# s3prl/s3prl

Hardware: AMD Instinct MI355X
Metric: encoder-frames/sec (20 ms stride) HuBERT-base 32x10 s @16 kHz (higher is better)
Workload: dtype f32; 1 GPU; hubert_base random-init, 32x10 s @16 kHz per GPU, one UpstreamExpert.forward per step: all 13 hidden_states (fp32) written; utterances_per_gpu=32, global_batch=32, samples=160000, frames_per_utt=499, parallelism=dp1, lengths=equal, gather=none

## Files before the change

### include/s3enc.h

```cpp
#ifndef S3ENC_H
#define S3ENC_H

#include <stdint.h>

#ifdef __cplusplus
extern "C" {
#endif

#define S3ENC_VERSION 8
#define S3ENC_MAX_CONV 16
#define S3ENC_MAX_RES 4

typedef struct s3enc_encoder* s3enc_handle;

enum { S3ENC_HUBERT = 0, S3ENC_WAV2VEC2 = 1, S3ENC_WAVLM = 2,
       S3ENC_DISTILLER = 3,
       S3ENC_MULTIRES = 4,
       S3ENC_WAV2VEC = 5,
       S3ENC_CPC = 6,
       S3ENC_APC = 7,
       S3ENC_MOCKINGJAY = 8,
       S3ENC_DECOAR = 9,
       S3ENC_NPC = 10 };
enum { S3ENC_F32 = 0, S3ENC_BF16 = 1, S3ENC_F16 = 2,
// ... 171 lines not shown
    const float* feat_w;
} s3enc_forward_opts;
int s3enc_num_states(s3enc_handle h, int32_t selection, int32_t* n);
int s3enc_forward_ex(s3enc_handle h, const float* const* wavs, const int64_t* lengths, int32_t B, int64_t n_max,
                     const s3enc_forward_opts* opts, void* out, int64_t layer_stride, void* stream);

int s3enc_forward_aux(s3enc_handle h, const float* const* wavs, const int64_t* lengths, int32_t B, int64_t n_max,
                      const s3enc_forward_opts* opts, void* out, int64_t layer_stride, float* codewords, int64_t* codeids,
                      void* stream);

enum { S3ENC_STATUS_NONFINITE = 1, S3ENC_STATUS_PENDING = 1 << 30 };
int s3enc_forward_status(s3enc_handle h, int32_t wait, int32_t* status);

int s3enc_set_layer_events(s3enc_handle h, void* const* events, int32_t n);

typedef struct s3enc_comm_s* s3enc_comm;
int s3enc_comm_version(int32_t* version);
int s3enc_comm_unique_id(void* id128);
int s3enc_comm_init_rank(const void* id128, int32_t world, int32_t rank, int32_t device, s3enc_comm* out);
int s3enc_comm_info(s3enc_comm c, int32_t* world, int32_t* rank);
int s3enc_comm_allgather_states(s3enc_comm c, const void* send, int64_t send_state_stride, void* recv, int64_t recv_state_stride,
                                int32_t n_states, int64_t bytes_per_state, void* const* ready_events, void* stream);
#define S3ENC_EXCHANGE_COLLECTIVE 0
#define S3ENC_EXCHANGE_DIRECT 1
#define S3ENC_EXCHANGE_COPY 2
#define S3ENC_COPY_HANDLE_BYTES 256
int s3enc_comm_init_local(int32_t world, int32_t rank, int32_t device, s3enc_comm* out);
int s3enc_comm_copy_export(s3enc_comm c, void* recv_slab, int64_t bytes, void* handle_out);
int s3enc_comm_copy_attach(s3enc_comm c, const void* handles );
int s3enc_comm_copy_status(s3enc_comm c, int32_t* status);
int s3enc_comm_copy_release(s3enc_comm c, void* stream);
int s3enc_comm_exchange_states(s3enc_comm c, int32_t algo, const void* send, int64_t send_state_stride, void* recv,
                               int64_t recv_state_stride, int32_t n_states, int64_t bytes_per_state, void* const* ready_events,
                               void* stream);
int s3enc_comm_destroy(s3enc_comm c);

int s3enc_forward_padded(s3enc_handle h, const float* pcm, int64_t row_stride, const int64_t* lengths, int32_t B,
                         int64_t n_max, float* out, int64_t layer_stride, void* stream);

int s3enc_profile_enable(s3enc_handle h, int32_t on);
int s3enc_profile_reset(s3enc_handle h);
typedef struct s3enc_profile_entry {
    char name[48];
    int64_t launches;
    double ms;
    double flops;
    double bytes;
} s3enc_profile_entry;
int s3enc_profile_read(s3enc_handle h, s3enc_profile_entry* entries, int32_t max_entries, int32_t* n_entries);

int s3enc_debug_tap(s3enc_handle h, const char* name, float* host_out, int64_t max_elems, int64_t* n_elems);
int s3enc_debug_occupy_cus(int32_t workgroups, int32_t threads, double milliseconds, void* stream);
int s3enc_debug_clock_sample(uint64_t* out3_device, void* stream);

int s3enc_set_tuning(const char* key, int32_t value);
int s3enc_set_handle_tuning(s3enc_handle h, const char* key, int32_t value);


int s3enc_op_gemm(int32_t dtype, const void* A, int64_t lda, int64_t a_batch_stride, const void* W,
                  const float* bias, int32_t M, int32_t N, int32_t K, int32_t batches, int32_t act,
                  const float* residual, const int32_t* row_limit, float* out32, void* out16, int64_t ldo,
                  int64_t o_batch_stride, void* stream);

int s3enc_op_conv0(int32_t dtype, const float* const* wavs, const int64_t* lengths, int32_t B, int64_t n_max,
                   int32_t normalize, const float* w0, const float* bias, const float* gn_gamma, const float* gn_beta,
                   const float* ln_gamma, const float* ln_beta, int32_t C, int32_t stride, void* out, void* stream);
int s3enc_op_wavlm_gate(const float* x, const float* grep_w, const float* grep_b, const float* grep_a, int32_t B, int32_t T,
                        int32_t H, float* gate, void* stream);

int s3enc_op_layernorm(int32_t dtype, const float* x, const float* gamma, const float* beta, int32_t rows,
                       int32_t C, int32_t act, float* out32, void* out16, void* stream);

int s3enc_op_attention(int32_t dtype, const void* qkv, void* out, const int32_t* valid, int32_t B, int32_t T,
                       int32_t H, const float* bias_table, int32_t table_R, const float* gate, void* stream);

int s3enc_op_conformer_conv(const float* x, const float* taps, const float* shift, int32_t B, int32_t T, int32_t D, int32_t K,
                            float* out, void* stream);
int s3enc_op_relpos_attention(const float* qkv, float* out, const int32_t* valid, int32_t B, int32_t T, int32_t H, const float* P,
                              const float* qadd, void* stream);

int s3enc_op_gn1_apply(const float* x, const float* gamma, const float* beta, const float* res, float scale, int32_t log_compress,
                       int32_t B, int32_t rows, int32_t C, int32_t pad, int32_t pad_zero, float* dst, float* state, float* acc,
                       float acc_w, int32_t acc_norm, int32_t acc_init, void* stream);
int s3enc_op_argmax_gather(const float* scores, const float* table, int32_t shared, int64_t rows, int32_t G, int32_t V, int32_t Dv,
                           int64_t* ids, float* out, void* stream);

int s3enc_op_channelnorm_relu(const float* x, const float* gamma, const float* beta, int32_t B, int32_t rows, int32_t C,
                              int32_t pad, float* dst, float* state, void* stream);
int s3enc_op_rnn(int32_t cell, const float* pre, const float* w_hh_host, const float* b_hn, int32_t B, int32_t T, int32_t H,
                 int64_t ld_pre, float* out, int64_t ldo, void* stream);

int s3enc_op_rnn_len(int32_t cell, const float* pre, const float* w_hh_host, const float* b_hn, const int32_t* len_host,
                     const float* res, int64_t ld_res, int32_t B, int32_t T, int32_t H, int64_t ld_pre, float* out, int64_t ldo,
                     void* stream);

int s3enc_op_conv_taps(const float* x, const float* w_host, const float* bias, int32_t B, int32_t T, int32_t C, int32_t N, int32_t k,
                       int32_t mask, int32_t act, const float* res, int64_t ld_res, float* dst, int32_t dst_pad, int64_t ldo,
                       float* state, float* sum, int32_t sum_init, int32_t dense, void* stream);

int s3enc_op_lstm_bidir(const float* pre_fwd, const float* pre_bwd, const float* w_hh_fwd_host, const float* w_hh_bwd_host,
                        const int32_t* len_host, int32_t B, int32_t T, int32_t H, int64_t ld_pre, float* out, int64_t ldo,
                        void* stream);
int s3enc_pack_lstm_bidir_whh(const float* w_hh_host, int32_t H, float* out_host);

int s3enc_op_posconv(int32_t dtype, const float* x, const float* w_host, const float* bias, int32_t B, int32_t T, int32_t D,
                     int32_t G, int32_t K, float* out, void* stream);
// ... 38 lines not shown
```

### s3prl_amd/_lib.py

```python

from __future__ import annotations

import ctypes as C
import os

_HERE = os.path.dirname(os.path.abspath(__file__))
LIB_PATH = os.path.join(_HERE, "libs3enc.so")

S3ENC_MAX_CONV = 16
S3ENC_MAX_RES = 4
F32, BF16, F16, F32X3, F16X2 = 0, 1, 2, 3, 4
STATUS_NONFINITE, STATUS_PENDING = 1, 1 << 30
DTYPES = {"fp32": F32, "f32": F32, "float32": F32, "bf16": BF16, "bfloat16": BF16, "fp16": F16, "f16": F16,
          "float16": F16, "fp32x3": F32X3, "f32x3": F32X3, "bf16x3": F32X3,
          "fp16x2": F16X2, "f16x2": F16X2}
FAMILY = {"hubert": 0, "wav2vec2": 1, "wavlm": 2, "distiller": 3, "multires_hubert": 4, "wav2vec": 5, "cpc": 6, "apc": 7, "mockingjay": 8, "decoar": 9, "npc": 10}
CPC_NORM = {"layerNorm": 0, "instanceNorm": 1, "ID": 2, "batchNorm": 3}
CPC_AR = {"LSTM": 0, "GRU": 1, "RNN": 2, "transformer": 3, "no_ar": 4}
APC_WINDOW = {"povey": 0, "hamming": 1}
VQ_TYPE = {"none": 0, "gumbel": 1, "kmeans": 2}
SEL_HIDDEN, SEL_LAYER_OUT, SEL_FFN_OUT = 0, 1, 2
SELECTIONS = {None: SEL_HIDDEN, "hidden_states": SEL_HIDDEN, "fairseq_layers": SEL_LAYER_OUT,
              "fairseq_layers_before_residual": SEL_FFN_OUT}
ABI_VERSION = 8
# ... 85 lines not shown

class S3FbankConfig(C.Structure):
    _fields_ = [("sample_rate", C.c_int32), ("num_mel_bins", C.c_int32), ("frame_length_ms", C.c_float),
                ("frame_shift_ms", C.c_float), ("preemphasis", C.c_float), ("delta_order", C.c_int32),
                ("delta_win_length", C.c_int32), ("use_cmvn", C.c_int32), ("cmvn_eps", C.c_float)]


_VP, _I32, _I64 = C.c_void_p, C.c_int32, C.c_int64
_PROTOS = {
    "s3enc_version": (C.c_int, []),
    "s3enc_last_error": (C.c_char_p, []),
    "s3enc_create": (C.c_int, [C.POINTER(S3Config), C.POINTER(S3Tensor), _I32, _I32, C.POINTER(_VP)]),
    "s3enc_create_ex": (C.c_int, [C.POINTER(S3Config), C.POINTER(S3Wav2vecConfig), C.POINTER(S3Tensor), _I32, _I32, C.POINTER(_VP)]),
    "s3enc_create_cpc": (C.c_int, [C.POINTER(S3Config), C.POINTER(S3CpcConfig), C.POINTER(S3Tensor), _I32, _I32, C.POINTER(_VP)]),
    "s3enc_create_apc": (C.c_int, [C.POINTER(S3Config), C.POINTER(S3ApcConfig), C.POINTER(S3Tensor), _I32, _I32, C.POINTER(_VP)]),
    "s3enc_create_mockingjay": (C.c_int, [C.POINTER(S3Config), C.POINTER(S3MockingjayConfig), C.POINTER(S3Tensor), _I32, _I32,
                                          C.POINTER(_VP)]),
    "s3enc_create_decoar": (C.c_int, [C.POINTER(S3Config), C.POINTER(S3DecoarConfig), C.POINTER(S3Tensor), _I32, _I32, C.POINTER(_VP)]),
    "s3enc_create_npc": (C.c_int, [C.POINTER(S3Config), C.POINTER(S3NpcConfig), C.POINTER(S3Tensor), _I32, _I32, C.POINTER(_VP)]),
    "s3enc_destroy": (C.c_int, [_VP]),
    "s3enc_num_frames": (C.c_int, [_VP, _I64, C.POINTER(_I32)]),
    "s3enc_num_output_frames": (C.c_int, [_VP, _I64, C.POINTER(_I32)]),
    "s3enc_downsample_rate": (C.c_int, [_VP, C.POINTER(_I32)]),
    "s3enc_valid_frames": (C.c_int, [_VP, _I64, _I64, C.POINTER(_I32)]),
    "s3enc_forward": (C.c_int, [_VP, C.POINTER(_VP), C.POINTER(_I64), _I32, _I64, _VP, _I64, _VP]),
    "s3enc_forward_status": (C.c_int, [_VP, _I32, C.POINTER(_I32)]),
    "s3enc_forward_ex": (C.c_int, [_VP, C.POINTER(_VP), C.POINTER(_I64), _I32, _I64, C.POINTER(S3ForwardOpts), _VP, _I64, _VP]),
    "s3enc_forward_aux": (C.c_int, [_VP, C.POINTER(_VP), C.POINTER(_I64), _I32, _I64, C.POINTER(S3ForwardOpts), _VP, _I64, _VP, _VP, _VP]),
    "s3enc_num_states": (C.c_int, [_VP, _I32, C.POINTER(_I32)]),
    "s3enc_forward_padded": (C.c_int, [_VP, _VP, _I64, C.POINTER(_I64), _I32, _I64, _VP, _I64, _VP]),
    "s3enc_set_layer_events": (C.c_int, [_VP, C.POINTER(_VP), _I32]),
    "s3enc_profile_enable": (C.c_int, [_VP, _I32]),
    "s3enc_profile_reset": (C.c_int, [_VP]),
    "s3enc_profile_read": (C.c_int, [_VP, C.POINTER(S3ProfileEntry), _I32, C.POINTER(_I32)]),
    "s3enc_debug_tap": (C.c_int, [_VP, C.c_char_p, C.POINTER(C.c_float), _I64, C.POINTER(_I64)]),
    "s3enc_comm_version": (C.c_int, [C.POINTER(_I32)]),
    "s3enc_comm_unique_id": (C.c_int, [_VP]),
    "s3enc_comm_init_rank": (C.c_int, [_VP, _I32, _I32, _I32, C.POINTER(_VP)]),
    "s3enc_comm_info": (C.c_int, [_VP, C.POINTER(_I32), C.POINTER(_I32)]),
    "s3enc_comm_allgather_states": (C.c_int, [_VP, _VP, _I64, _VP, _I64, _I32, _I64, C.POINTER(_VP), _VP]),
    "s3enc_comm_exchange_states": (C.c_int, [_VP, _I32, _VP, _I64, _VP, _I64, _I32, _I64, C.POINTER(_VP), _VP]),
    "s3enc_comm_destroy": (C.c_int, [_VP]),
    "s3enc_comm_init_local": (C.c_int, [_I32, _I32, _I32, C.POINTER(_VP)]),
    "s3enc_comm_copy_export": (C.c_int, [_VP, _VP, _I64, _VP]),
    "s3enc_comm_copy_attach": (C.c_int, [_VP, _VP]),
    "s3enc_comm_copy_status": (C.c_int, [_VP, C.POINTER(_I32)]),
    "s3enc_comm_copy_release": (C.c_int, [_VP, _VP]),
    "s3enc_set_handle_tuning": (C.c_int, [_VP, C.c_char_p, _I32]),
    "s3enc_set_tuning": (C.c_int, [C.c_char_p, _I32]),
    "s3enc_op_gemm": (C.c_int, [_I32, _VP, _I64, _I64, _VP, _VP, _I32, _I32, _I32, _I32, _I32, _VP, _VP, _VP, _VP,
                                _I64, _I64, _VP]),
    "s3enc_debug_occupy_cus": (C.c_int, [_I32, _I32, C.c_double, _VP]),
    "s3enc_debug_clock_sample": (C.c_int, [_VP, _VP]),
    "s3enc_op_layernorm": (C.c_int, [_I32, _VP, _VP, _VP, _I32, _I32, _I32, _VP, _VP, _VP]),
    "s3enc_op_attention": (C.c_int, [_I32, _VP, _VP, _VP, _I32, _I32, _I32, _VP, _I32, _VP, _VP]),
    "s3enc_op_conv0": (C.c_int, [_I32, C.POINTER(_VP), C.POINTER(_I64), _I32, _I64, _I32, _VP, _VP, _VP, _VP, _VP, _VP, _I32,
                                 _I32, _VP, _VP]),
    "s3enc_op_wavlm_gate": (C.c_int, [_VP, _VP, _VP, _VP, _I32, _I32, _I32, _VP, _VP]),
    "s3enc_op_conformer_conv": (C.c_int, [_VP, _VP, _VP, _I32, _I32, _I32, _I32, _VP, _VP]),
    "s3enc_op_gn1_apply": (C.c_int, [_VP, _VP, _VP, _VP, C.c_float, _I32, _I32, _I32, _I32, _I32, _I32, _VP, _VP, _VP, C.c_float,
                                     _I32, _I32, _VP]),
    "s3enc_op_channelnorm_relu": (C.c_int, [_VP, _VP, _VP, _I32, _I32, _I32, _I32, _VP, _VP, _VP]),
    "s3enc_op_rnn": (C.c_int, [_I32, _VP, _VP, _VP, _I32, _I32, _I32, _I64, _VP, _I64, _VP]),
    "s3enc_op_rnn_len": (C.c_int, [_I32, _VP, _VP, _VP, _VP, _VP, _I64, _I32, _I32, _I32, _I64, _VP, _I64, _VP]),
    "s3enc_op_lstm_bidir": (C.c_int, [_VP, _VP, _VP, _VP, _VP, _I32, _I32, _I32, _I64, _VP, _I64, _VP]),
    "s3enc_pack_lstm_bidir_whh": (C.c_int, [_VP, _I32, _VP]),
    "s3enc_op_conv_taps": (C.c_int, [_VP, _VP, _VP, _I32, _I32, _I32, _I32, _I32, _I32, _I32, _VP, _I64, _VP, _I32, _I64, _VP, _VP,
                                     _I32, _I32, _VP]),
    "s3enc_op_argmax_gather": (C.c_int, [_VP, _VP, _I32, _I64, _I32, _I32, _I32, _VP, _VP, _VP]),
    "s3enc_op_relpos_attention": (C.c_int, [_VP, _VP, _VP, _I32, _I32, _I32, _VP, _VP, _VP]),
    "s3enc_op_posconv": (C.c_int, [_I32, _VP, _VP, _VP, _I32, _I32, _I32, _I32, _I32, _VP, _VP]),
    "s3enc_weighted_sum": (C.c_int, [_VP, _I64, _I32, C.POINTER(C.c_float), _I32, _I64, _I32, _VP, _VP]),
    "s3enc_weighted_sum_backward_scratch": (_I64, [_I64, _I32]),
    "s3enc_weighted_sum_backward": (C.c_int, [_VP, _I64, _I32, _I32, _I64, _I32, _VP, _VP, _VP, _VP]),
    "s3enc_fbank_num_frames": (C.c_int, [C.POINTER(S3FbankConfig), _I64, C.POINTER(_I32)]),
    "s3enc_fbank_forward": (C.c_int, [C.POINTER(S3FbankConfig), _VP, C.POINTER(_I64), _I32, _VP, _I64, _I32, _VP]),
    "s3enc_fbank_forward_ex": (C.c_int, [C.POINTER(S3FbankConfig), _I32, _VP, C.POINTER(_I64), _I32, _VP, _I64, _I32, _VP]),
    "s3enc_logmel_frame_counts": (C.c_int, [C.POINTER(_I64), _I32, _I64, C.POINTER(_I32)]),
    "s3enc_logmel_forward": (C.c_int, [_VP, C.POINTER(_I64), _I32, _I64, _I32, C.c_float, _I32, C.POINTER(_I32), _VP, _I32, _VP]),
    "s3enc_op_layernorm_eps": (C.c_int, [_VP, _VP, _VP, C.c_float, _I64, _I32, _VP, _VP]),
    "s3enc_op_input_repr": (C.c_int, [_VP, _VP, _VP, _VP, _I32, _VP, _VP, C.c_float, _I64, _I32, _I32, _VP, _VP]),
}

_lib = None


class S3EncError(RuntimeError):
    pass


def load():
    global _lib
    if _lib is not None:
        return _lib
    if not os.path.exists(LIB_PATH):
        raise S3EncError(
            f"{LIB_PATH} not found — build it with `python -c 'import __graft_entry__ as g; g.build()'` "
            f"or `make -C s3prl_amd/csrc`.  There is no CPU / PyTorch fallback for the encoder path."
        )
    try:
        import torch
    except Exception:
        pass
    lib = C.CDLL(LIB_PATH, mode=C.RTLD_GLOBAL)
    for name, (res, args) in _PROTOS.items():
        fn = getattr(lib, name)
# ... 164 lines not shown
```

### s3prl_amd/csrc/gemmt.hip

```cpp
#include <type_traits>

#include "kernels.h"

namespace s3 {

namespace {

constexpr int BN = 128, ROWB = 64;
typedef int i32x4 __attribute__((ext_vector_type(4)));

struct x3_tag {};
template <typename T> struct TileElem { typedef typename Cvt<T>::store_t type; };
template <> struct TileElem<x3_tag> { typedef float type; };

template <typename T> struct TileMma;
template <> struct TileMma<float> {
    static __device__ __forceinline__ void run(const uint4& a, const uint4& b, f32x16& c) {
        c = __builtin_amdgcn_mfma_f32_32x32x2f32(__uint_as_float(a.x), __uint_as_float(b.x), c, 0, 0, 0);
        c = __builtin_amdgcn_mfma_f32_32x32x2f32(__uint_as_float(a.y), __uint_as_float(b.y), c, 0, 0, 0);
        c = __builtin_amdgcn_mfma_f32_32x32x2f32(__uint_as_float(a.z), __uint_as_float(b.z), c, 0, 0, 0);
        c = __builtin_amdgcn_mfma_f32_32x32x2f32(__uint_as_float(a.w), __uint_as_float(b.w), c, 0, 0, 0);
    }
};
template <> struct TileMma<bf16_tag> {
    static __device__ __forceinline__ void run(const uint4& a, const uint4& b, f32x16& c) {
        c = __builtin_amdgcn_mfma_f32_32x32x16_bf16(__builtin_bit_cast(bf16x8, a), __builtin_bit_cast(bf16x8, b), c, 0, 0, 0);
    }
};
template <typename T, int TM>
__global__ __launch_bounds__(256, 2) void gemm_tile_kernel(GemmParams p) {
    typedef typename TileElem<T>::type store_t;
    constexpr int EB = sizeof(store_t);
    constexpr bool X3 = std::is_same<T, x3_tag>::value;
    constexpr int BM = 64 * TM;
    constexpr int PLANE = (BM + BN) * ROWB;
    constexpr int NPASS = (BM + BN) / 64;
    constexpr int APASS = BM / 64;
    extern __shared__ __attribute__((aligned(16))) char smem[];
    const int tid = threadIdx.x;
    const int lane = tid & 63;
    const int wave = __builtin_amdgcn_readfirstlane(tid >> 6);
    const int wr = wave >> 1, wc = wave & 1;
    const int half = lane >> 5;
    const int l31 = lane & 31;

    const int n_tiles = (p.N + BN - 1) / BN;
    const int m_tiles = (p.M + BM - 1) / BM;
    int tile;
    {
        const int nwg = gridDim.x, wg = blockIdx.x;
        const int q8 = nwg >> 3, r8 = nwg & 7, xcd = wg & 7, loc = wg >> 3;
        tile = (xcd < r8 ? xcd * (q8 + 1) : r8 * (q8 + 1) + (xcd - r8) * q8) + loc;
    }
    const int tn = tile % n_tiles;
    const int tmb = tile / n_tiles;
    const int tm = tmb % m_tiles, b = tmb / m_tiles;
    const int m0 = tm * BM, n0 = tn * BN;
    const int nk = (p.K * EB) >> 6;

    i32x4 rsrc_a, rsrc_w;
    {
        const char* ab = (const char*)p.A + (long)b * p.a_bs * EB;
        const unsigned long ua = (unsigned long)ab, uw = (unsigned long)(X3 ? p.W_x3 : p.W);
        rsrc_a = (i32x4){(int)__builtin_amdgcn_readfirstlane((unsigned)ua), (int)__builtin_amdgcn_readfirstlane((unsigned)(ua >> 32)),
                         -1, 0x00020000};
        rsrc_w = (i32x4){(int)__builtin_amdgcn_readfirstlane((unsigned)uw), (int)__builtin_amdgcn_readfirstlane((unsigned)(uw >> 32)),
                         -1, 0x00020000};
    }
    const int src_slot = (lane & 3) ^ ((lane >> 4) & 3);
    unsigned voff[NPASS];
#pragma unroll
    for (int i = 0; i < NPASS; ++i) {
        if (i < APASS) {
            int r = m0 + 16 * wave + 64 * i + (lane >> 2);
            r = r < p.M ? r : p.M - 1;
            voff[i] = (unsigned)r * (unsigned)(p.lda * EB) + src_slot * 16;
        } else {
            int r = n0 + 16 * wave + 64 * (i - APASS) + (lane >> 2);
            r = r < p.N ? r : p.N - 1;
            voff[i] = (unsigned)r * (unsigned)(p.K * EB) + src_slot * 16;
        }
    }
    const unsigned lds0 = __builtin_amdgcn_readfirstlane((unsigned)(uintptr_t)(__attribute__((address_space(3))) char*)smem) + wave * 1024;
    auto dma = [&](unsigned vo, const i32x4& rs, unsigned dst, unsigned soff) {
        asm volatile("s_mov_b32 m0, %0\n\ts_nop 0\n\tbuffer_load_dwordx4 %1, %2, %3 offen lds"
                     :
                     : "s"(dst), "v"(vo), "s"(rs), "s"(soff)
                     : "memory");
    };
    auto issue = [&](int kt, int slot) {
        const unsigned kb = (unsigned)kt * ROWB;
        const unsigned d0 = lds0 + slot * PLANE;
#pragma unroll
        for (int i = 0; i < NPASS; ++i) dma(voff[i], i < APASS ? rsrc_a : rsrc_w, d0 + i * 4096, kb);
    };

    const int swz = (l31 >> 2) & 3;
    const char* fa_base = smem + (wr * (TM * 32) + l31) * ROWB;
    const char* fb_base = smem + (BM + wc * 64 + l31) * ROWB;
    const int so0 = ((half * 2) ^ swz) << 4, so1 = ((half * 2 + 1) ^ swz) << 4;

    f32x16 acc[TM][2];
#pragma unroll
    for (int i = 0; i < TM; ++i)
#pragma unroll
        for (int j = 0; j < 2; ++j)
#pragma unroll
            for (int r = 0; r < 16; ++r) acc[i][j][r] = 0.f;

    struct Frag {
        uint4 a[TM], b[2];
    };
    auto read = [&](Frag& f, int slot, int so) {
#pragma unroll
        for (int i = 0; i < TM; ++i) f.a[i] = *(const uint4*)(fa_base + slot * PLANE + i * 32 * ROWB + so);
#pragma unroll
        for (int j = 0; j < 2; ++j) f.b[j] = *(const uint4*)(fb_base + slot * PLANE + j * 32 * ROWB + so);
    };
    issue(0, 0);
    asm volatile("s_waitcnt vmcnt(0)" ::: "memory");
    __builtin_amdgcn_s_barrier();
    asm volatile("" ::: "memory");
    if (nk > 1) issue(1, 1);
    if constexpr (!X3) {
        auto mma = [&](const Frag& f, int i, int j) { TileMma<T>::run(f.a[i], f.b[j], acc[i][j]); };
        auto mma_all = [&](const Frag& f) {
#pragma unroll
            for (int i = 0; i < TM; ++i)
#pragma unroll
                for (int j = 0; j < 2; ++j) mma(f, i, j);
        };
        Frag f0, f1;
        read(f0, 0, so0);
        auto step = [&](int kt, int slot) {
            read(f1, slot, so1);
            mma_all(f0);
            __builtin_amdgcn_sched_barrier(0);
            asm volatile("s_waitcnt vmcnt(0) lgkmcnt(0)" ::: "memory");
            __builtin_amdgcn_s_barrier();
            asm volatile("" ::: "memory");
            __builtin_amdgcn_sched_barrier(0);
            mma(f1, 0, 0);
            __builtin_amdgcn_sched_barrier(0);
            if (kt + 2 < nk) issue(kt + 2, slot);
            if (kt + 1 < nk) read(f0, slot ^ 1, so0);
            __builtin_amdgcn_sched_barrier(0);
#pragma unroll
            for (int i = 0; i < TM; ++i)
#pragma unroll
                for (int j = 0; j < 2; ++j)
                    if (i | j) mma(f1, i, j);
        };
        int kt = 0;
        for (; kt + 1 < nk; kt += 2) {
            step(kt, 0);
            step(kt + 1, 1);
        }
        if (kt < nk) step(kt, 0);
    } else {
        auto mma_row = [&](const Frag& lo_half, const Frag& hi_half, int i) {
            uint4 ah, al;
            split8(__builtin_bit_cast(float4, lo_half.a[i]), __builtin_bit_cast(float4, hi_half.a[i]), ah, al);
#pragma unroll
            for (int j = 0; j < 2; ++j) {
                TileMma<bf16_tag>::run(al, lo_half.b[j], acc[i][j]);
                TileMma<bf16_tag>::run(ah, hi_half.b[j], acc[i][j]);
                TileMma<bf16_tag>::run(ah, lo_half.b[j], acc[i][j]);
            }
        };
        Frag f0, f1, g0, g1;
        read(f0, 0, so0);
        read(f1, 0, so1);
        auto step = [&](int kt, int slot, Frag& c0, Frag& c1, Frag& n0_, Frag& n1_) {
            mma_row(c0, c1, 0);
            __builtin_amdgcn_sched_barrier(0);
            asm volatile("s_waitcnt vmcnt(0) lgkmcnt(0)" ::: "memory");
            __builtin_amdgcn_s_barrier();
            asm volatile("" ::: "memory");
            __builtin_amdgcn_sched_barrier(0);
            if (kt + 2 < nk) issue(kt + 2, slot);
            if (kt + 1 < nk) {
                read(n0_, slot ^ 1, so0);
                read(n1_, slot ^ 1, so1);
            }
            __builtin_amdgcn_sched_barrier(0);
#pragma unroll
            for (int i = 1; i < TM; ++i) mma_row(c0, c1, i);
        };
        int kt = 0;
        for (; kt + 1 < nk; kt += 2) {
            step(kt, 0, f0, f1, g0, g1);
            step(kt + 1, 1, g0, g1, f0, f1);
        }
        if (kt < nk) step(kt, 0, f0, f1, g0, g1);
    }

    const int limit = p.row_limit ? p.row_limit[b] : p.M;
    const long ob = (long)b * p.o_bs;
    float* stg = (float*)(smem + wave * 8192);
    {
        const int c4 = (lane & 15) * 4;
        const int n = n0 + wc * 64 + c4;
        const bool n_ok = n < p.N;
        float4 bias4 = make_float4(0.f, 0.f, 0.f, 0.f);
        if (p.bias && n_ok) bias4 = *(const float4*)(p.bias + n);
#pragma unroll
        for (int i = 0; i < TM; ++i) {
#pragma unroll
            for (int j = 0; j < 2; ++j)
#pragma unroll
                for (int r = 0; r < 16; ++r) stg[((r & 3) + 8 * (r >> 2) + 4 * half) * 64 + j * 32 + l31] = acc[i][j][r];
            asm volatile("s_waitcnt lgkmcnt(0)" ::: "memory");
#pragma unroll
            for (int t = 0; t < 8; ++t) {
                const int row = t * 4 + (lane >> 4);
                float4 v = *(const float4*)(stg + row * 64 + c4);
                const int m = m0 + wr * (TM * 32) + i * 32 + row;
                if (m < p.M && n_ok) {
                    v.x += bias4.x; v.y += bias4.y; v.z += bias4.z; v.w += bias4.w;
                    if (p.act == 3) {
                        swish4(v);
                    } else if (p.act) {
                        if (X3 || p.act == 2) {
                            gelu_fast4(v);
                        } else {
                            v.x = gelu_erf(v.x); v.y = gelu_erf(v.y); v.z = gelu_erf(v.z); v.w = gelu_erf(v.w);
                        }
                    }
                    const long o = ob + (long)m * p.ldo + n;
                    if (p.residual) {
                        const float4 rs = *(const float4*)(p.residual + o);
                        v.x += rs.x; v.y += rs.y; v.z += rs.z; v.w += rs.w;
                    }
                    if (m >= limit) v = make_float4(0.f, 0.f, 0.f, 0.f);
                    *(float4*)(p.out32 + o) = v;
                }
            }
            asm volatile("s_waitcnt lgkmcnt(0)" ::: "memory");
        }
    }
}

template <typename T, int TM>
hipError_t go(const GemmParams& p, hipStream_t stream) {
    constexpr int BM = 64 * TM;
    constexpr int plane2 = 2 * (BM + BN) * ROWB;
    constexpr int lds = plane2 > 4 * 8192 ? plane2 : 4 * 8192;
    hipError_t e = ensure_dynamic_lds<gemm_tile_kernel<T, TM>>(lds);
    if (e != hipSuccess) return e;
    dim3 grid(((p.M + BM - 1) / BM) * ((p.N + BN - 1) / BN) * p.batches);
    hipLaunchKernelGGL((gemm_tile_kernel<T, TM>), grid, dim3(256), lds, stream, p);
    return hipGetLastError();
}
template <typename T>
hipError_t go_tm(int tm, const GemmParams& p, hipStream_t stream) {
    switch (tm) {
        case 4: return go<T, 4>(p, stream);
        case 3: return go<T, 3>(p, stream);
        case 2: return go<T, 2>(p, stream);
        case 1: return go<T, 1>(p, stream);
    }
    return hipErrorInvalidValue;
}

double tile_efficiency(const GemmParams& p, int tm, int cus) {
    const long bm = 64L * tm;
    const long mt = (p.M + bm - 1) / bm, nt = (p.N + BN - 1) / BN;
    const long tiles = mt * nt * p.batches;
    const double cover = ((double)p.M * p.N) / ((double)mt * bm * nt * BN);
    const long per_cu = (tiles + cus - 1) / cus;
    const double balance = (double)tiles / ((double)per_cu * cus);
    double steady = 1.0;
    if (tm == 1) steady = 0.90;
    if (tm == 3) steady = 0.988;
    if (tm == 4) steady = p.K >= 6144 ? 1.01 : 0.965;
    return cover * balance * steady;
}

}

int device_cus() {
    static int cus = 0;
    if (!cus) {
        int dev = 0, n = 0;
        if (hipGetDevice(&dev) == hipSuccess && hipDeviceGetAttribute(&n, hipDeviceAttributeMultiprocessorCount, dev) == hipSuccess && n > 0)
            cus = n;
        else
            cus = 256;
    }
    return cus;
}

int gemm_tile_pick(int mode, const GemmParams& p) {
    const int cus = device_cus();
    if (mode >= 2) return 6 - mode;
    int best = 0;
    double best_e = 0.0;
    for (int tm = 2; tm <= 4; ++tm) {
        const double e = tile_efficiency(p, tm, cus);
        if (e > best_e + 1e-9) {
            best_e = e;
            best = tm;
        }
    }
    if (best_e < 0.5) {
        const double e = tile_efficiency(p, 1, cus);
        if (e > best_e + 1e-9) best = 1;
    }
    return best;
}

bool gemm_tile_eligible(int dtype, const GemmParams& p) {
    if (dtype != F32 && dtype != 3) return false;
    const int mode = dtype == F32 ? tuning().gemm32_big : tuning().gemm_x3_tile;
    if (!mode || !p.out32 || p.out16) return false;
    if (dtype == 3 && !p.W_x3) return false;
    if ((p.K & 15) || (p.N & 3) || (p.ldo & 3) || (p.o_bs & 3) || ((p.lda * 4) & 15) || ((p.a_bs * 4) & 15)) return false;
    const uintptr_t al = (uintptr_t)p.A | (uintptr_t)(dtype == 3 ? p.W_x3 : p.W) | (uintptr_t)p.out32 | (uintptr_t)p.residual |
                         (uintptr_t)p.bias;
    if (al & 15) return false;
    if (p.M < 64 || p.N < 128) return false;
    const unsigned long a_span = ((unsigned long)(p.M - 1) * (unsigned long)p.lda + (unsigned long)p.K) * 4ul;
    const unsigned long w_span = (unsigned long)p.N * (unsigned long)p.K * 4ul;
    if (a_span >= (1ul << 32) - 64 || w_span >= (1ul << 32) - 64) return false;
    if (dtype == 3 && mode == 1) {
        const long t256 = (long)((p.M + 255) / 256) * ((p.N + 255) / 256) * p.batches;
        if (t256 * 2 > device_cus()) return false;
    }
    return gemm_tile_pick(mode, p) != 0;
}

hipError_t launch_gemm_tile(int dtype, const GemmParams& p, hipStream_t stream) {
    const int tm = gemm_tile_pick(dtype == F32 ? tuning().gemm32_big : tuning().gemm_x3_tile, p);
    return dtype == 3 ? go_tm<x3_tag>(tm, p, stream) : go_tm<float>(tm, p, stream);
}

}
```

### s3prl_amd/csrc/kernels.h

```cpp
#pragma once
#include <cstring>
#include <vector>

#include "common.h"

namespace s3 {
int device_cus();

template <auto Kern>
inline hipError_t ensure_dynamic_lds(int bytes) {
    static int granted[64] = {};
    int dev = 0;
    hipError_t e = hipGetDevice(&dev);
    if (e != hipSuccess) return e;
    if (dev >= 0 && dev < 64 && granted[dev] >= bytes) return hipSuccess;
    e = hipFuncSetAttribute((const void*)Kern, hipFuncAttributeMaxDynamicSharedMemorySize, bytes);
    if (e == hipSuccess && dev >= 0 && dev < 64) granted[dev] = bytes;
    return e;
}

struct Tuning {
    int gemm_variant = 3;
    int gemm_lds_pad = 0;
    int gemm32_big = 1;
    int gemm_x3_tile = 1;
    int gemm16_big = 3;
    int gemm16_pp = 0;
    int gemm16_mx = 14;
    int reserve_cus = 0;
    int gemm16_rows = 1;
    int attn_lds_pad = 0;
    int attn_persist = 0;
    int conv0_nt = 1;
    int conv_f22 = 1;
    int conv0_fast = 1;
    int ws_inplace = 1;
    int gelu32 = 1;
    int x3_pack_cache = 0;
    int fp16x2_conv1_f32 = 0;
    int ln_rows = 1;
    int ln_preload = 1;
    int ln1_fold = 1;
    int gn_lag_one_block = 1;
    int forward_chain = 1;
    int rnn_split = -1;
    int npc_skip_taps = 1;
    int comm_self_p2p = 0;
};
extern Tuning g_tuning;
extern thread_local const Tuning* t_tuning;
inline const Tuning& tuning() { return t_tuning ? *t_tuning : g_tuning; }
struct TuningScope {
    const Tuning* prev;
    explicit TuningScope(const Tuning* t) : prev(t_tuning) { if (t) t_tuning = t; }
    ~TuningScope() { t_tuning = prev; }
};
int tuning_set(Tuning& t, const char* key, int value, const char** err);

extern thread_local int* t_status;
struct StatusScope {
    int* prev;
    explicit StatusScope(int* p) : prev(t_status) { t_status = p; }
    ~StatusScope() { t_status = prev; }
};

struct GemmParams {
    const void* A;
    long lda, a_bs;
    const void* W;
    const void* W_x3 = nullptr;
    const float* bias;
    int M, N, K, batches;
    int act;
    const float* residual;
    const int* row_limit;
    const float2* res_ln_stats = nullptr;
    const float* res_ln_g = nullptr;
    const float* res_ln_b = nullptr;
    float* out32;
    void* out16;
    long ldo, o_bs;
    int variant = -1;
    long ldw = 0;
    int wsplit = 0;
    const void* W4 = nullptr;
    const void* W4s = nullptr;
    int mxw = 0;
};
bool gemm16_mx_eligible(int dtype, const GemmParams& p);
bool gemm16_mx_weight_rule(long N, long K);
bool gemm_x3_eligible(const GemmParams& p);
hipError_t launch_gemm_x3(const GemmParams& p, hipStream_t stream);
void pack_x3(const float* w, long N, long K, std::vector<uint16_t>& out);
bool gemm16_big_eligible(int dtype, const GemmParams& p);
bool gemm16_res_ln_ok(int dtype, const GemmParams& p);
hipError_t launch_gemm16_big(int dtype, const GemmParams& p, hipStream_t stream);
bool gemm_tile_eligible(int dtype, const GemmParams& p);
hipError_t launch_gemm_tile(int dtype, const GemmParams& p, hipStream_t stream);
hipError_t launch_gemm(int dtype, const GemmParams& p, hipStream_t stream);
struct ConvF22Params {
    const float* x;
    long x_bs;
    const float* W;
    const float* WP;
    const float* bias;
    int M, C, batches;
    int act;
    const int* row_limit;
    float* out;
    long o_bs;
};
bool conv_f22_eligible(const ConvF22Params& p);
hipError_t launch_conv_f22(const ConvF22Params& p, hipStream_t stream);
struct ConvTapsParams {
    const float* src;
    long src_bs;
    int C;
    const float* W;
    const float* bias;
    int T, N, B;
    int taps0, gap, taps1;
    int act;
    const float* res;
    long res_bs, ld_res;
    float* dst;
    long dst_bs, ld_dst;
    float* state;
    long state_bs, ld_state;
    float* sum;
    long sum_bs, ld_sum;
    int sum_init;
};
void pack_conv_taps(const float* w, int N, int C, int k, int mask, bool dense, std::vector<float>& out);
const char* conv_taps_refusal(const ConvTapsParams& p);
hipError_t launch_conv_taps(const ConvTapsParams& p, hipStream_t stream);

struct WavTable {
    const float* const* ptrs;
    const long* lens;
    int B;
    long n_max;
};
constexpr int STAT_K0_MAX = 16;
hipError_t launch_wav_norm_stats(const WavTable& w, int normalize, double* partial, float2* norm, hipStream_t s,
                                 float eps = 0.f );
hipError_t launch_gn_stats(const WavTable& w, const float2* norm, const float* w0 , const float* gamma,
                           const float* beta, int C, int k0, int s0, long L0, double* partial, double* sums,
                           float2* gn, hipStream_t s);
size_t stats_partial_elems(int B, long n_max);
struct Conv0Params {
// ... 289 lines not shown
```

### s3prl_amd/csrc/ops.hip

```cpp
#include "engine_internal.h"

namespace s3 {
Tuning g_tuning;
thread_local const Tuning* t_tuning = nullptr;
thread_local int* t_status = nullptr;

int tuning_set(Tuning& t, const char* key, int value, const char** err) {
    struct Key {
        const char* name;
        int Tuning::*field;
        int lo, hi;
    };
    static const Key keys[] = {
        {"gemm_variant", &Tuning::gemm_variant, 0, 63},      {"gemm_lds_pad", &Tuning::gemm_lds_pad, 0, 120 * 1024},
        {"gemm32_big", &Tuning::gemm32_big, 0, 5},           {"gemm_x3_tile", &Tuning::gemm_x3_tile, 0, 5},
        {"gemm16_big", &Tuning::gemm16_big, 0, 10},          {"gemm16_rows", &Tuning::gemm16_rows, 0, 1},
        {"attn_lds_pad", &Tuning::attn_lds_pad, 0, 48 * 1024}, {"conv0_nt", &Tuning::conv0_nt, 0, 1},
        {"ws_inplace", &Tuning::ws_inplace, 0, 1},           {"gemm16_pp", &Tuning::gemm16_pp, 0, 3},
        {"gemm16_mx", &Tuning::gemm16_mx, 0, 31},            {"reserve_cus", &Tuning::reserve_cus, 0, 128},
        {"x3_pack_cache", &Tuning::x3_pack_cache, 0, 1},     {"gelu32", &Tuning::gelu32, 0, 1},
        {"comm_self_p2p", &Tuning::comm_self_p2p, 0, 1},     {"attn_persist", &Tuning::attn_persist, 0, 1},
        {"fp16x2_conv1_f32", &Tuning::fp16x2_conv1_f32, 0, 1}, {"gn_lag_one_block", &Tuning::gn_lag_one_block, 0, 1},
        {"ln_rows", &Tuning::ln_rows, 1, 2},                 {"ln1_fold", &Tuning::ln1_fold, 0, 1},
        {"ln_preload", &Tuning::ln_preload, 0, 1},           {"forward_chain", &Tuning::forward_chain, 0, 1},
        {"conv0_fast", &Tuning::conv0_fast, 0, 1},           {"conv_f22", &Tuning::conv_f22, 0, 1},
        {"rnn_split", &Tuning::rnn_split, -1, 8},           {"npc_skip_taps", &Tuning::npc_skip_taps, 0, 1},
    };
    static thread_local char msg[160];
    if (!key) {
        *err = "s3enc_set_tuning: null key";
        return 1;
    }
    for (const Key& k : keys)
        if (!strcmp(key, k.name)) {
            if (value < k.lo || value > k.hi) {
                snprintf(msg, sizeof(msg), "%s must be %d..%d", k.name, k.lo, k.hi);
                *err = msg;
                return 1;
            }
            t.*(k.field) = value;
            return 0;
        }
    snprintf(msg, sizeof(msg), "s3enc_set_tuning: unknown key '%s'", key);
    *err = msg;
    return 1;
}
}

extern "C" {

int s3enc_set_tuning(const char* key, int32_t value) {
    const char* err = nullptr;
    if (tuning_set(g_tuning, key, value, &err)) return fail(err);
    return 0;
}
int s3enc_set_handle_tuning(s3enc_handle h, const char* key, int32_t value) {
    if (!h) return fail("null handle");
    if (!h->has_tuning) {
        h->tun = g_tuning;
        h->has_tuning = true;
    }
    const char* err = nullptr;
    if (tuning_set(h->tun, key, value, &err)) return fail(err);
    return 0;
}

int s3enc_op_gemm(int32_t dtype, const void* A, int64_t lda, int64_t a_batch_stride, const void* W, const float* bias, int32_t M,
                  int32_t N, int32_t K, int32_t batches, int32_t act, const float* residual, const int32_t* row_limit,
                  float* out32, void* out16, int64_t ldo, int64_t o_batch_stride, void* stream) {
    GemmParams g{};
    g.A = A;
    g.lda = lda;
    g.a_bs = a_batch_stride;
    g.W = W;
    g.bias = bias;
    g.M = M;
    g.N = N;
    g.K = K;
    g.batches = batches;
// ... 49 lines not shown
        HIP_TRY(launch_gemm(F32, g, (hipStream_t)stream));
        HIP_TRY(hipStreamSynchronize((hipStream_t)stream));
        if (tuning().x3_pack_cache) {
            HIP_TRY(hipDeviceSynchronize());
            std::swap(cached.p, w3.p);
            std::swap(cached.bytes, w3.bytes);
            cached_w = W;
            cached_n = N;
            cached_k = K;
        }
        return 0;
    }
    HIP_TRY(launch_gemm(dtype, g, (hipStream_t)stream));
    return 0;
}

namespace {
__global__ void occupy_kernel(long long ticks) {
    const long long t0 = wall_clock64();
    while (wall_clock64() - t0 < ticks) __builtin_amdgcn_s_sleep(32);
}
}
int s3enc_debug_occupy_cus(int32_t workgroups, int32_t threads, double milliseconds, void* stream) {
    if (workgroups <= 0 || threads <= 0 || threads > 1024 || !(milliseconds >= 0) || milliseconds > 10000.0)
        return fail("s3enc_debug_occupy_cus: bad argument (workgroups > 0, 0 < threads <= 1024, 0 <= milliseconds <= 10000)");
    int dev = 0, khz = 0;
    HIP_TRY(hipGetDevice(&dev));
    if (hipDeviceGetAttribute(&khz, hipDeviceAttributeWallClockRate, dev) != hipSuccess || khz <= 0) khz = 100000;
    hipLaunchKernelGGL(occupy_kernel, dim3(workgroups), dim3(threads), 0, (hipStream_t)stream, (long long)(milliseconds * khz));
    HIP_TRY(hipGetLastError());
    return 0;
}

namespace {
__global__ void clock_sample_kernel(unsigned long long* out, unsigned long long ref_khz) {
    if (threadIdx.x) return;
    const unsigned xcc = __builtin_amdgcn_s_getreg((3 << 11) | 20) & 15u;
    if (xcc != 0) return;
    if (atomicCAS(&out[2], 0ull, ref_khz) != 0ull) return;
    out[0] = __builtin_amdgcn_s_memtime();
    out[1] = __builtin_amdgcn_s_memrealtime();
    __threadfence_system();
}
}
int s3enc_debug_clock_sample(uint64_t* out3_device, void* stream) {
    if (!out3_device) return fail("s3enc_debug_clock_sample: null argument");
    int dev = 0, khz = 0;
    HIP_TRY(hipGetDevice(&dev));
    if (hipDeviceGetAttribute(&khz, hipDeviceAttributeWallClockRate, dev) != hipSuccess || khz <= 0) khz = 100000;
    HIP_TRY(hipMemsetAsync(out3_device, 0, 3 * sizeof(uint64_t), (hipStream_t)stream));
    hipLaunchKernelGGL(clock_sample_kernel, dim3(64), dim3(64), 0, (hipStream_t)stream, (unsigned long long*)out3_device,
                       (unsigned long long)khz);
    HIP_TRY(hipGetLastError());
    return 0;
}

int s3enc_op_layernorm(int32_t dtype, const float* x, const float* gamma, const float* beta, int32_t rows, int32_t C, int32_t act,
                       float* out32, void* out16, void* stream) {
    HIP_TRY(launch_layernorm(dtype, x, gamma, beta, rows, C, act, out32, out16, (hipStream_t)stream));
    return 0;
}

int s3enc_op_attention(int32_t dtype, const void* qkv, void* out, const int32_t* valid, int32_t B, int32_t T, int32_t H,
                       const float* bias_table, int32_t table_R, const float* gate, void* stream) {
    if (bias_table && (table_R < 0 || T > 6000)) return fail("s3enc_op_attention: bad table_R / T > 6000 with a bias table");
    AttnParams a{};
    a.qkv = qkv;
    a.out = out;
    a.valid = valid;
    a.B = B;
    a.T = T;
    a.H = H;
    a.bias_table = bias_table;
    a.table_R = table_R;
    a.gate = gate;
    HIP_TRY(launch_attention(dtype, a, (hipStream_t)stream));
    return 0;
}

int s3enc_op_conformer_conv(const float* x, const float* taps, const float* shift, int32_t B, int32_t T, int32_t D, int32_t K,
                            float* out, void* stream) {
    if (!x || !taps || !shift || !out) return fail("s3enc_op_conformer_conv: null argument");
    if (B <= 0 || T <= 0 || D <= 0 || D % 64) return fail("s3enc_op_conformer_conv: bad shape (D % 64 == 0)");
    if (K < 1 || K > 63 || !(K & 1)) return fail("s3enc_op_conformer_conv: K must be odd and <= 63");
    ConformerConvParams p{};
    p.x = x;
    p.taps = taps;
    p.shift = shift;
    p.out = out;
    p.B = B;
    p.T = T;
    p.D = D;
    p.K = K;
    HIP_TRY(launch_conformer_conv(p, (hipStream_t)stream));
    return 0;
}

int s3enc_op_gn1_apply(const float* x, const float* gamma, const float* beta, const float* res, float scale, int32_t log_compress,
                       int32_t B, int32_t rows, int32_t C, int32_t pad, int32_t pad_zero, float* dst, float* state, float* acc,
                       float acc_w, int32_t acc_norm, int32_t acc_init, void* stream) {
    if (!x || (!dst && !state && !acc)) return fail("s3enc_op_gn1_apply: null argument");
    if (B <= 0 || rows <= 0 || C <= 0 || (C & 3) || C > 1024) return fail("s3enc_op_gn1_apply: bad shape (C % 4 == 0, C <= 1024)");
    if (pad < 0 || pad > 64 || (pad && !dst)) return fail("s3enc_op_gn1_apply: pad rows need dst (0..64)");
    hipStream_t st = (hipStream_t)stream;
    double* partial = nullptr;
    HIP_TRY(hipMalloc((void**)&partial, (size_t)B * GS_BLOCKS * 2 * sizeof(double)));
// ... 563 lines not shown
```

Measured before the change: 463,000 frames/s.

## Split fp32 tile GEMM into tall bulk tiles plus 64-row tail tiles

Adds a wave-quantization-aware schedule to the fp32 tile GEMM. It keeps tall TM×64-row tiles for the bulk of M and covers the leftover rows with single-64-row tail tiles when a cost model predicts a partial last wave. Tail tiles are handed out per XCD after the bulk tiles. The epilogue now prefetches residual rows ahead of use, double-buffered per row block. This adds a second template instantiation, more register pressure for the residual prefetch, and a heuristic model with hard-coded occupancy constants.

```diff
diff --git a/include/s3enc.h b/include/s3enc.h
--- a/include/s3enc.h
+++ b/include/s3enc.h
@@ -247,6 +247,8 @@
 int s3enc_debug_tap(s3enc_handle h, const char* name, float* host_out, int64_t max_elems, int64_t* n_elems);
 int s3enc_debug_occupy_cus(int32_t workgroups, int32_t threads, double milliseconds, void* stream);
 int s3enc_debug_clock_sample(uint64_t* out3_device, void* stream);
+int s3enc_debug_gemm_schedule(int32_t M, int32_t N, int32_t batches, int32_t tm, int32_t tail, int32_t cus, int32_t* items4_host,
+                              int64_t max_items, int64_t* n_items);
 
 int s3enc_set_tuning(const char* key, int32_t value);
 int s3enc_set_handle_tuning(s3enc_handle h, const char* key, int32_t value);
diff --git a/s3prl_amd/_lib.py b/s3prl_amd/_lib.py
--- a/s3prl_amd/_lib.py
+++ b/s3prl_amd/_lib.py
@@ -161,6 +161,7 @@
                                 _I64, _I64, _VP]),
     "s3enc_debug_occupy_cus": (C.c_int, [_I32, _I32, C.c_double, _VP]),
     "s3enc_debug_clock_sample": (C.c_int, [_VP, _VP]),
+    "s3enc_debug_gemm_schedule": (C.c_int, [_I32, _I32, _I32, _I32, _I32, _I32, _VP, _I64, C.POINTER(_I64)]),
     "s3enc_op_layernorm": (C.c_int, [_I32, _VP, _VP, _VP, _I32, _I32, _I32, _VP, _VP, _VP]),
     "s3enc_op_attention": (C.c_int, [_I32, _VP, _VP, _VP, _I32, _I32, _I32, _VP, _I32, _VP, _VP]),
     "s3enc_op_conv0": (C.c_int, [_I32, C.POINTER(_VP), C.POINTER(_I64), _I32, _I64, _I32, _VP, _VP, _VP, _VP, _VP, _VP, _I32,
diff --git a/s3prl_amd/csrc/gemmt.hip b/s3prl_amd/csrc/gemmt.hip
--- a/s3prl_amd/csrc/gemmt.hip
+++ b/s3prl_amd/csrc/gemmt.hip
@@ -1,3 +1,4 @@
+#include <algorithm>
 #include <type_traits>
 
 #include "kernels.h"
@@ -27,15 +28,37 @@
         c = __builtin_amdgcn_mfma_f32_32x32x16_bf16(__builtin_bit_cast(bf16x8, a), __builtin_bit_cast(bf16x8, b), c, 0, 0, 0);
     }
 };
-template <typename T, int TM>
-__global__ __launch_bounds__(256, 2) void gemm_tile_kernel(GemmParams p) {
+struct TileItem {
+    int b, m0, n0;
+    bool tail;
+};
+__host__ __device__ inline TileItem tile_item(int wg, int nwg, int n_tiles, int batches, int bm, int m_bulk, int m_tail) {
+    const int nb = m_bulk * n_tiles * batches;
+    const int xcd = wg & 7, loc = wg >> 3;
+    const int q8 = nwg >> 3, r8 = nwg & 7, qb = nb >> 3, rb = nb & 7;
+    const int start = xcd < r8 ? xcd * (q8 + 1) : r8 * (q8 + 1) + (xcd - r8) * q8;
+    const int bstart = xcd < rb ? xcd * (qb + 1) : rb * (qb + 1) + (xcd - rb) * qb;
+    const int bcnt = qb + (xcd < rb ? 1 : 0);
+    TileItem it;
+    it.tail = loc >= bcnt;
+    const int tile = it.tail ? (start - bstart) + (loc - bcnt) : bstart + loc;
+    const int mt = it.tail ? m_tail : m_bulk;
+    const int tn = tile % n_tiles, tmb = tile / n_tiles;
+    it.b = tmb / mt;
+    it.m0 = it.tail ? m_bulk * bm + (tmb % mt) * 64 : (tmb % mt) * bm;
+    it.n0 = tn * BN;
+    return it;
+}
+
+template <typename T, int TM, int TE>
+__device__ __forceinline__ void tile_body(const GemmParams& p, const int b, const int m0, const int n0) {
     typedef typename TileElem<T>::type store_t;
     constexpr int EB = sizeof(store_t);
     constexpr bool X3 = std::is_same<T, x3_tag>::value;
     constexpr int BM = 64 * TM;
     constexpr int PLANE = (BM + BN) * ROWB;
-    constexpr int NPASS = (BM + BN) / 64;
-    constexpr int APASS = BM / 64;
+    constexpr int NPASS = TE + BN / 64;
+    constexpr int APASS = TE;
     extern __shared__ __attribute__((aligned(16))) char smem[];
     const int tid = threadIdx.x;
     const int lane = tid & 63;
@@ -43,19 +66,6 @@
     const int wr = wave >> 1, wc = wave & 1;
     const int half = lane >> 5;
     const int l31 = lane & 31;
-
-    const int n_tiles = (p.N + BN - 1) / BN;
-    const int m_tiles = (p.M + BM - 1) / BM;
-    int tile;
-    {
-        const int nwg = gridDim.x, wg = blockIdx.x;
-        const int q8 = nwg >> 3, r8 = nwg & 7, xcd = wg & 7, loc = wg >> 3;
-        tile = (xcd < r8 ? xcd * (q8 + 1) : r8 * (q8 + 1) + (xcd - r8) * q8) + loc;
-    }
-    const int tn = tile % n_tiles;
-    const int tmb = tile / n_tiles;
-    const int tm = tmb % m_tiles, b = tmb / m_tiles;
-    const int m0 = tm * BM, n0 = tn * BN;
     const int nk = (p.K * EB) >> 6;
 
     i32x4 rsrc_a, rsrc_w;
@@ -92,28 +102,28 @@
         const unsigned kb = (unsigned)kt * ROWB;
         const unsigned d0 = lds0 + slot * PLANE;
 #pragma unroll
-        for (int i = 0; i < NPASS; ++i) dma(voff[i], i < APASS ? rsrc_a : rsrc_w, d0 + i * 4096, kb);
+        for (int i = 0; i < NPASS; ++i) dma(voff[i], i < APASS ? rsrc_a : rsrc_w, d0 + (i < APASS ? i : i - APASS + TM) * 4096, kb);
     };
 
     const int swz = (l31 >> 2) & 3;
-    const char* fa_base = smem + (wr * (TM * 32) + l31) * ROWB;
+    const char* fa_base = smem + (wr * (TE * 32) + l31) * ROWB;
     const char* fb_base = smem + (BM + wc * 64 + l31) * ROWB;
     const int so0 = ((half * 2) ^ swz) << 4, so1 = ((half * 2 + 1) ^ swz) << 4;
 
-    f32x16 acc[TM][2];
-#pragma unroll
-    for (int i = 0; i < TM; ++i)
+    f32x16 acc[TE][2];
+#pragma unroll
+    for (int i = 0; i < TE; ++i)
 #pragma unroll
         for (int j = 0; j < 2; ++j)
 #pragma unroll
             for (int r = 0; r < 16; ++r) acc[i][j][r] = 0.f;
 
     struct Frag {
-        uint4 a[TM], b[2];
+        uint4 a[TE], b[2];
     };
     auto read = [&](Frag& f, int slot, int so) {
 #pragma unroll
-        for (int i = 0; i < TM; ++i) f.a[i] = *(const uint4*)(fa_base + slot * PLANE + i * 32 * ROWB + so);
+        for (int i = 0; i < TE; ++i) f.a[i] = *(const uint4*)(fa_base + slot * PLANE + i * 32 * ROWB + so);
 #pragma unroll
         for (int j = 0; j < 2; ++j) f.b[j] = *(const uint4*)(fb_base + slot * PLANE + j * 32 * ROWB + so);
     };
@@ -126,7 +136,7 @@
         auto mma = [&](const Frag& f, int i, int j) { TileMma<T>::run(f.a[i], f.b[j], acc[i][j]); };
         auto mma_all = [&](const Frag& f) {
 #pragma unroll
-            for (int i = 0; i < TM; ++i)
+            for (int i = 0; i < TE; ++i)
 #pragma unroll
                 for (int j = 0; j < 2; ++j) mma(f, i, j);
         };
@@ -146,7 +156,7 @@
             if (kt + 1 < nk) read(f0, slot ^ 1, so0);
             __builtin_amdgcn_sched_barrier(0);
 #pragma unroll
-            for (int i = 0; i < TM; ++i)
+            for (int i = 0; i < TE; ++i)
 #pragma unroll
                 for (int j = 0; j < 2; ++j)
                     if (i | j) mma(f1, i, j);
@@ -185,7 +195,7 @@
             }
             __builtin_amdgcn_sched_barrier(0);
 #pragma unroll
-            for (int i = 1; i < TM; ++i) mma_row(c0, c1, i);
+            for (int i = 1; i < TE; ++i) mma_row(c0, c1, i);
         };
         int kt = 0;
         for (; kt + 1 < nk; kt += 2) {
@@ -195,6 +205,8 @@
         if (kt < nk) step(kt, 0, f0, f1, g0, g1);
     }
 
+    constexpr bool PRE = !X3;
+    constexpr bool AHEAD = TE != 3;
     const int limit = p.row_limit ? p.row_limit[b] : p.M;
     const long ob = (long)b * p.o_bs;
     float* stg = (float*)(smem + wave * 8192);
@@ -204,18 +216,30 @@
         const bool n_ok = n < p.N;
         float4 bias4 = make_float4(0.f, 0.f, 0.f, 0.f);
         if (p.bias && n_ok) bias4 = *(const float4*)(p.bias + n);
-#pragma unroll
-        for (int i = 0; i < TM; ++i) {
+        float4 res[2][8];
+        auto load_res = [&](int i, float4 (&r)[8]) {
+#pragma unroll
+            for (int t = 0; t < 8; ++t) {
+                const int m = m0 + wr * (TE * 32) + i * 32 + t * 4 + (lane >> 4);
+                r[t] = make_float4(0.f, 0.f, 0.f, 0.f);
+                if (m < p.M && n_ok) r[t] = *(const float4*)(p.residual + ob + (long)m * p.ldo + n);
+            }
+        };
+        if (PRE && AHEAD && p.residual) load_res(0, res[0]);
+#pragma unroll
+        for (int i = 0; i < TE; ++i) {
 #pragma unroll
             for (int j = 0; j < 2; ++j)
 #pragma unroll
                 for (int r = 0; r < 16; ++r) stg[((r & 3) + 8 * (r >> 2) + 4 * half) * 64 + j * 32 + l31] = acc[i][j][r];
+            if (PRE && !AHEAD && i == 0 && p.residual) load_res(0, res[0]);
+            if (PRE && AHEAD && i + 1 < TE && p.residual) load_res(i + 1, res[(i + 1) & 1]);
             asm volatile("s_waitcnt lgkmcnt(0)" ::: "memory");
 #pragma unroll
             for (int t = 0; t < 8; ++t) {
                 const int row = t * 4 + (lane >> 4);
                 float4 v = *(const float4*)(stg + row * 64 + c4);
-                const int m = m0 + wr * (TM * 32) + i * 32 + row;
+                const int m = m0 + wr * (TE * 32) + i * 32 + row;
                 if (m < p.M && n_ok) {
                     v.x += bias4.x; v.y += bias4.y; v.z += bias4.z; v.w += bias4.w;
                     if (p.act == 3) {
@@ -229,36 +253,51 @@
                     }
                     const long o = ob + (long)m * p.ldo + n;
                     if (p.residual) {
-                        const float4 rs = *(const float4*)(p.residual + o);
+                        const float4 rs = PRE ? res[i & 1][t] : *(const float4*)(p.residual + o);
                         v.x += rs.x; v.y += rs.y; v.z += rs.z; v.w += rs.w;
                     }
                     if (m >= limit) v = make_float4(0.f, 0.f, 0.f, 0.f);
                     *(float4*)(p.out32 + o) = v;
                 }
             }
+            if (PRE && !AHEAD && i + 1 < TE && p.residual) load_res(i + 1, res[(i + 1) & 1]);
             asm volatile("s_waitcnt lgkmcnt(0)" ::: "memory");
         }
     }
 }
 
 template <typename T, int TM>
-hipError_t go(const GemmParams& p, hipStream_t stream) {
+__global__ __launch_bounds__(256, 2) void gemm_tile_kernel(GemmParams p, int m_bulk, int m_tail) {
+    constexpr bool MIX = TM > 1 && !std::is_same<T, x3_tag>::value;
+    const int n_tiles = (p.N + BN - 1) / BN;
+    const TileItem it = tile_item(blockIdx.x, gridDim.x, n_tiles, p.batches, 64 * TM, m_bulk, MIX ? m_tail : 0);
+    if constexpr (MIX) {
+        if (it.tail) {
+            tile_body<T, TM, 1>(p, it.b, it.m0, it.n0);
+            return;
+        }
+    }
+    tile_body<T, TM, TM>(p, it.b, it.m0, it.n0);
+}
+
+template <typename T, int TM>
+hipError_t go(const GemmParams& p, const GemmTileSched& s, hipStream_t stream) {
     constexpr int BM = 64 * TM;
     constexpr int plane2 = 2 * (BM + BN) * ROWB;
     constexpr int lds = plane2 > 4 * 8192 ? plane2 : 4 * 8192;
     hipError_t e = ensure_dynamic_lds<gemm_tile_kernel<T, TM>>(lds);
     if (e != hipSuccess) return e;
-    dim3 grid(((p.M + BM - 1) / BM) * ((p.N + BN - 1) / BN) * p.batches);
-    hipLaunchKernelGGL((gemm_tile_kernel<T, TM>), grid, dim3(256), lds, stream, p);
+    dim3 grid((s.m_bulk + s.m_tail) * ((p.N + BN - 1) / BN) * p.batches);
+    hipLaunchKernelGGL((gemm_tile_kernel<T, TM>), grid, dim3(256), lds, stream, p, s.m_bulk, s.m_tail);
     return hipGetLastError();
 }
 template <typename T>
-hipError_t go_tm(int tm, const GemmParams& p, hipStream_t stream) {
-    switch (tm) {
-        case 4: return go<T, 4>(p, stream);
-        case 3: return go<T, 3>(p, stream);
-        case 2: return go<T, 2>(p, stream);
-        case 1: return go<T, 1>(p, stream);
+hipError_t go_tm(const GemmParams& p, const GemmTileSched& s, hipStream_t stream) {
+    switch (s.tm) {
+        case 4: return go<T, 4>(p, s, stream);
+        case 3: return go<T, 3>(p, s, stream);
+        case 2: return go<T, 2>(p, s, stream);
+        case 1: return go<T, 1>(p, s, stream);
     }
     return hipErrorInvalidValue;
 }
@@ -277,6 +316,57 @@
     return cover * balance * steady;
 }
 
+constexpr int tile_resident(int tm) { return tm >= 4 ? 2 : tm == 3 ? 3 : 4; }
+constexpr double kAloneTall[5] = {0, 0.77, 0.91, 0.91, 0.92};
+constexpr double kAloneTail = 0.77;
+constexpr double kTailSteady = 0.95;
+constexpr double kTailMargin = 1.05;
+double occupancy(int k, int r, double alone) { return k >= r ? 1.0 : 1.0 - (1.0 - alone) * (double)(r - k) / (double)(r - 1); }
+double rounds_cost(long k, int r, double units, double alone) {
+    const long whole = k / r, rest = k % r;
+    return (double)whole * r * units + (rest ? (double)rest * units / occupancy((int)rest, r, alone) : 0.0);
+}
+
+}
+
+GemmTileSched gemm_tile_schedule(int M, int N, int batches, int tm, int tail_mode, int tail_units, int cus) {
+    const int bm = 64 * tm;
+    GemmTileSched s{tm, (M + bm - 1) / bm, 0};
+    if (!tail_mode || tm < 2) return s;
+    const long per_m = (long)((N + BN - 1) / BN) * batches;
+    int m_bulk;
+    if (tail_mode == 2) {
+        m_bulk = M > bm ? 1 : 0;
+    } else if (tail_units > 0) {
+        m_bulk = M > 64 * tail_units ? (M - 64 * tail_units) / bm : 0;
+    } else {
+        const int r = tile_resident(tm);
+        const long slots = (long)cus * r, tiles = s.m_bulk * per_m;
+        const long whole = tiles / slots, rest = tiles % slots;
+        if (!whole || !rest) return s;
+        m_bulk = (int)std::min<long>(whole * slots / per_m, M / bm);
+        const long m_tail = (M - m_bulk * bm + 63) / 64;
+        const long past = m_tail * per_m - (whole * slots - m_bulk * per_m);
+        const double with_tail = past > 0 ? rounds_cost((past + cus - 1) / cus, r, 1.0 / kTailSteady, kAloneTail) : 0.0;
+        const double without = rounds_cost((rest + cus - 1) / cus, r, tm, kAloneTall[tm]);
+        if (with_tail * kTailMargin >= without) return s;
+    }
+    if (m_bulk * bm >= M) return s;
+    s.m_bulk = m_bulk;
+    s.m_tail = (M - m_bulk * bm + 63) / 64;
+    return s;
+}
+
+void gemm_tile_items(int M, int N, int batches, const GemmTileSched& s, std::vector<int>& items4) {
+    const int n_tiles = (N + BN - 1) / BN, bm = 64 * s.tm;
+    const int nwg = (s.m_bulk + s.m_tail) * n_tiles * batches;
+    items4.clear();
+    items4.reserve((size_t)nwg * 4);
+    for (int wg = 0; wg < nwg; ++wg) {
+        const TileItem it = tile_item(wg, nwg, n_tiles, batches, bm, s.m_bulk, s.m_tail);
+        const int rows = std::min(it.tail ? 64 : bm, M - it.m0);
+        items4.insert(items4.end(), {it.b, it.m0, rows, it.n0});
+    }
 }
 
 int device_cus() {
@@ -332,7 +422,8 @@
 
 hipError_t launch_gemm_tile(int dtype, const GemmParams& p, hipStream_t stream) {
     const int tm = gemm_tile_pick(dtype == F32 ? tuning().gemm32_big : tuning().gemm_x3_tile, p);
-    return dtype == 3 ? go_tm<x3_tag>(tm, p, stream) : go_tm<float>(tm, p, stream);
-}
-
-}
+    if (dtype == 3) return go_tm<x3_tag>(p, gemm_tile_schedule(p.M, p.N, p.batches, tm, 0, 0, device_cus()), stream);
+    return go_tm<float>(p, gemm_tile_schedule(p.M, p.N, p.batches, tm, tuning().gemm32_tail, tuning().gemm32_tail_units, device_cus()), stream);
+}
+
+}
diff --git a/s3prl_amd/csrc/kernels.h b/s3prl_amd/csrc/kernels.h
--- a/s3prl_amd/csrc/kernels.h
+++ b/s3prl_amd/csrc/kernels.h
@@ -24,6 +24,8 @@
     int gemm_lds_pad = 0;
     int gemm32_big = 1;
     int gemm_x3_tile = 1;
+    int gemm32_tail = 1;
+    int gemm32_tail_units = 0;
     int gemm16_big = 3;
     int gemm16_pp = 0;
     int gemm16_mx = 14;
@@ -96,6 +98,11 @@
 bool gemm16_res_ln_ok(int dtype, const GemmParams& p);
 hipError_t launch_gemm16_big(int dtype, const GemmParams& p, hipStream_t stream);
 bool gemm_tile_eligible(int dtype, const GemmParams& p);
+struct GemmTileSched {
+    int tm, m_bulk, m_tail;
+};
+GemmTileSched gemm_tile_schedule(int M, int N, int batches, int tm, int tail_mode, int tail_units, int cus);
+void gemm_tile_items(int M, int N, int batches, const GemmTileSched& s, std::vector<int>& items4);
 hipError_t launch_gemm_tile(int dtype, const GemmParams& p, hipStream_t stream);
 hipError_t launch_gemm(int dtype, const GemmParams& p, hipStream_t stream);
 struct ConvF22Params {
diff --git a/s3prl_amd/csrc/ops.hip b/s3prl_amd/csrc/ops.hip
--- a/s3prl_amd/csrc/ops.hip
+++ b/s3prl_amd/csrc/ops.hip
@@ -25,6 +25,7 @@
         {"ln_preload", &Tuning::ln_preload, 0, 1},           {"forward_chain", &Tuning::forward_chain, 0, 1},
         {"conv0_fast", &Tuning::conv0_fast, 0, 1},           {"conv_f22", &Tuning::conv_f22, 0, 1},
         {"rnn_split", &Tuning::rnn_split, -1, 8},           {"npc_skip_taps", &Tuning::npc_skip_taps, 0, 1},
+        {"gemm32_tail", &Tuning::gemm32_tail, 0, 2},         {"gemm32_tail_units", &Tuning::gemm32_tail_units, 0, 1 << 20},
     };
     static thread_local char msg[160];
     if (!key) {
@@ -180,6 +181,19 @@
     hipLaunchKernelGGL(clock_sample_kernel, dim3(64), dim3(64), 0, (hipStream_t)stream, (unsigned long long*)out3_device,
                        (unsigned long long)khz);
     HIP_TRY(hipGetLastError());
+    return 0;
+}
+
+int s3enc_debug_gemm_schedule(int32_t M, int32_t N, int32_t batches, int32_t tm, int32_t tail, int32_t cus, int32_t* items4_host,
+                              int64_t max_items, int64_t* n_items) {
+    if (!n_items) return fail("s3enc_debug_gemm_schedule: null argument");
+    if (M < 1 || N < 1 || batches < 1 || tm < 1 || tm > 4 || tail < 0 || tail > 2 || cus < 1)
+        return fail("s3enc_debug_gemm_schedule: M, N, batches, cus >= 1, tm 1..4, tail 0..2");
+    const GemmTileSched s = gemm_tile_schedule(M, N, batches, tm, tail, 0, cus);
+    std::vector<int> items;
+    gemm_tile_items(M, N, batches, s, items);
+    *n_items = (int64_t)(items.size() / 4);
+    if (items4_host && max_items >= *n_items) memcpy(items4_host, items.data(), items.size() * sizeof(int));
     return 0;
 }
 
```

Result: faster. 467,900 frames/s, median of 6 (+1.0%).
